# facebookresearch/metamorph

Hardware: AMD Instinct MI355X
Metric: train tokens/sec (LLaMA-3-8B + SigLIP-SO400M, seq2048, 256 img toks), whole job (higher is better)
Workload: dtype bf16

## Files before the change

metamorph_amd/csrc/attn.hip:

```cpp
#include "mm355_common.h"
#include "attn2.h"
#include <cstdlib>
#include <algorithm>

namespace {

constexpr int NT = 256;

__global__ __launch_bounds__(NT) void attn_delta_kernel(const uint16_t* __restrict__ o, const uint16_t* __restrict__ d_o, int64_t ld_o,
                                                        float* __restrict__ delta, int L, int Hq, int d) {
    const int l = blockIdx.x * 64 + (threadIdx.x >> 2), part = threadIdx.x & 3;
    const int h = blockIdx.y, b = blockIdx.z;
    const int dv = d >> 3;
    float s = 0.f;
    if (l < L) {
        for (int v = part; v < dv; v += 4) {
            float x[8], y[8];
            unpack8(*(const u32x4*)(o + ((int64_t)b * L + l) * ld_o + (int64_t)h * d + v * 8), x);
            unpack8(*(const u32x4*)(d_o + ((int64_t)b * L + l) * ld_o + (int64_t)h * d + v * 8), y);
#pragma unroll
            for (int e = 0; e < 8; ++e) s += x[e] * y[e];
        }
    }
    s += __shfl_xor(s, 1, 64);
// ... 72 lines not shown
    (void)hipGetLastError();
    if (!o || !d_o || !delta || B <= 0 || L <= 0 || Hq <= 0 || d <= 0 || d > 128 || (d & 7) || (ld_o & 7)) return MM355_EINVAL;
    dim3 grid((unsigned)((L + 63) / 64), (unsigned)Hq, (unsigned)B);
    hipLaunchKernelGGL(attn_delta_kernel, grid, dim3(NT), 0, (hipStream_t)stream, o, d_o, ld_o, delta, (int)L, (int)Hq, (int)d);
    return mm_launch_status();
}

extern "C" int64_t mm355_attn_bwd_ws_floats(int64_t B, int64_t L, int64_t Hq, int64_t Hkv, int64_t d, int64_t ld_max) {
    if (fast128(d, ld_max)) return 2 * B * Hq * L;
    if (Hq == Hkv) return 0;
    return 2 * B * L * Hq * d;
}

namespace {
int attn_bwd_impl(const mm355_bf16* q, const mm355_bf16* k, const mm355_bf16* v, int64_t ld_q, int64_t ld_k, const mm355_bf16* d_o,
                  int64_t ld_o, const float* lse, const float* delta, const int32_t* seqlens, mm355_bf16* dq, int64_t ld_dq,
                  mm355_bf16* dk, mm355_bf16* dv, int64_t ld_dkv, int64_t B, int64_t L, int64_t Hq, int64_t Hkv, int64_t d,
                  float scale, int causal, float* workspace, const uint16_t* rope_cos, const uint16_t* rope_sin, const int32_t* rope_pos,
                  int variant, void* stream) {
    (void)hipGetLastError();
    if (!q || !k || !v || !d_o || !lse || !delta || !dq || !dk || !dv || bad_geom(B, L, Hq, Hkv, d)) return MM355_EINVAL;
    if ((ld_q & 7) || (ld_k & 7) || (ld_o & 7) || (ld_dkv & 7) || (ld_dq & 7)) return MM355_EINVAL;
    const int64_t ld_max = std::max(std::max(ld_q, ld_k), ld_o);
    if (variant == 3) return MM355_EUNSUPPORTED;
    if (variant != 0 && variant != 2 && variant != 4 && variant != 41) return MM355_EINVAL;
    const bool is128 = fast128(d, ld_max) && variant != 2;
    const bool can4 = is128 && workspace && L * ld_max * 2 < 0x7fffffffll;
    if (is128 && !can4 && Hq != Hkv) return workspace ? MM355_EUNSUPPORTED : MM355_EINVAL;
    if (rope_cos && !can4) return MM355_EUNSUPPORTED;
    if ((variant == 4 || variant == 41) && !can4) return MM355_EUNSUPPORTED;
    if (variant == 4 || variant == 41 || (variant == 0 && can4)) {
        attn2::Args a4{q, k, v, d_o, ld_q, ld_k, ld_o, nullptr, nullptr, lse, delta, dq, ld_dq, seqlens,
                       dk, dv, nullptr, nullptr, ld_dkv, (int)B, (int)L, (int)Hq, (int)Hkv, (int)d, scale, causal, rope_cos, rope_sin, rope_pos};
        return mm355_attn4_bwd_launch(a4, workspace, variant == 41, (hipStream_t)stream);
    }
    if (Hq != Hkv && !workspace) return MM355_EINVAL;
    hipStream_t s = (hipStream_t)stream;
    float* dkp = nullptr;
    float* dvp = nullptr;
    if (Hq != Hkv) {
        dkp = workspace;
        dvp = workspace + (int64_t)B * L * Hq * d;
    }
    attn2::Args a{q, k, v, d_o, ld_q, ld_k, ld_o, nullptr, nullptr, lse, delta, dq, ld_dq, seqlens,
                  dk, dv, dkp, dvp, ld_dkv, (int)B, (int)L, (int)Hq, (int)Hkv, (int)d, scale, causal, rope_cos, rope_sin, rope_pos};
    int rc = mm355_attn2_dkdv_launch(a, pick_dp(d), s);
    if (rc != MM355_OK) return rc;
    if (dkp) {
        const int64_t rows = B * L;
        const unsigned rg = (unsigned)std::min<int64_t>((rows * (Hkv * d / 8) + NT - 1) / NT, 4096);
        hipLaunchKernelGGL(group_reduce_kernel, dim3(rg), dim3(NT), 0, s, dkp, dk, ld_dkv, rows, (int)Hq, (int)Hkv, (int)d);
        hipLaunchKernelGGL(group_reduce_kernel, dim3(rg), dim3(NT), 0, s, dvp, dv, ld_dkv, rows, (int)Hq, (int)Hkv, (int)d);
        rc = mm_launch_status();
        if (rc != MM355_OK) return rc;
    }
    return mm355_attn2_dq_launch(a, pick_dp(d), s);
}
}

extern "C" int mm355_attn_bwd(const mm355_bf16* q, const mm355_bf16* k, const mm355_bf16* v, int64_t ld_q, int64_t ld_k, const mm355_bf16* d_o,
                              int64_t ld_o, const float* lse, const float* delta, const int32_t* seqlens, mm355_bf16* dq, int64_t ld_dq,
                              mm355_bf16* dk, mm355_bf16* dv, int64_t ld_dkv, int64_t B, int64_t L, int64_t Hq, int64_t Hkv, int64_t d,
                              float scale, int causal, float* workspace, void* stream) {
    return attn_bwd_impl(q, k, v, ld_q, ld_k, d_o, ld_o, lse, delta, seqlens, dq, ld_dq, dk, dv, ld_dkv, B, L, Hq, Hkv, d, scale, causal, workspace,
                         nullptr, nullptr, nullptr, 0, stream);
}

// ... 20 lines not shown
```

metamorph_amd/csrc/attn4_bwd.hip:

```cpp
#include "attn2.h"

#ifndef ATTN4B_GEN_DIR
#define ATTN4B_GEN_DIR attn4_bwd_gen
#endif
#define ATTN4B_STR2(x) #x
#define ATTN4B_STR(x) ATTN4B_STR2(x)
#define ATTN4B_INC(f) ATTN4B_STR(ATTN4B_GEN_DIR/f)

namespace attn4b {
using namespace attn2;

constexpr float LOG2E = 1.4426950408889634f;
constexpr int SLOT = 32768;
constexpr int KV_BASE = 2048;
constexpr int KV_LDS = KV_BASE + 4 * SLOT, Q_LDS = 4 * SLOT;

MM_DEV int rot4(int row) { return ((row & 3) << 2) | ((row >> 2) & 3); }

struct LaneAddr {
    int RA[8], TA[4], TB[4], SA;
    MM_DEV void init(int lane) {
        const int c = lane & 31, hi = lane >> 5, g = lane >> 4, i = lane & 15;
#pragma unroll
        for (int ks = 0; ks < 8; ++ks) RA[ks] = c * 256 + (((ks * 2 + hi) ^ rot4(c)) << 4);
        const int row0 = 4 * hi + (i >> 2), row1 = row0 + 8;
#pragma unroll
        for (int db = 0; db < 4; ++db) {
            const int chunk = db * 4 + (g & 1) * 2 + ((i & 3) >> 1);
            TA[db] = row0 * 256 + ((chunk ^ rot4(row0)) << 4) + (i & 1) * 8;
            TB[db] = row1 * 256 + ((chunk ^ rot4(row1)) << 4) + (i & 1) * 8;
        }
        SA = hi * 16;
    }
};
MM_DEV void piece_offsets(int wave, int lane, uint32_t ldb, uint32_t (&vo)[4]) {
    const int r4 = lane >> 4, pc = lane & 15;
#pragma unroll
    for (int i = 0; i < 4; ++i) vo[i] = (uint32_t)(16 * wave + 4 * i + r4) * ldb + (uint32_t)((pc ^ ((r4 << 2) | i)) << 4);
}
MM_DEV uint32_t scale_pair(uint32_t w, float s) { return pack2bf(bflo(w) * s, bfhi(w) * s); }

#define BWD_BARRIER() asm volatile("s_waitcnt vmcnt(%0)\n\ts_barrier" :: "n"(NDMA) : "memory")

template <bool SAFE>
__global__ __launch_bounds__(256, 1) __attribute__((amdgpu_num_vgpr(96))) void dkdv_kernel(Args a, const float* __restrict__ nstat) {
    extern __shared__ __attribute__((aligned(16))) unsigned char smem[];
    asm volatile("" ::: "v255", "a255");
#ifdef MM355_ATTN4_TIMING
// ... 441 lines not shown
                for (int r = 0; r < 4; ++r) hi_[r] = x_[r] * keep;
            }
            if (a.rope_cos) {
                const int col = dbp * 32 + 8 * i4_ + 4 * hi;
                const u32x2 cw = *(const u32x2*)(a.rope_cos + (int64_t)pos * 128 + col);
                const u32x2 sw = *(const u32x2*)(a.rope_sin + (int64_t)pos * 128 + col);
                const float cs[4] = {bflo(cw.x), bfhi(cw.x), bflo(cw.y), bfhi(cw.y)};
                const float sn[4] = {bflo(sw.x), bfhi(sw.x), bflo(sw.y), bfhi(sw.y)};
#pragma unroll
                for (int r = 0; r < 4; ++r) {
                    const float x1 = round_bf(lo_[r]), x2 = round_bf(hi_[r]);
                    lo_[r] = x1 * cs[r] + x2 * sn[r];
                    hi_[r] = x2 * cs[r] - x1 * sn[r];
                }
            }
#pragma unroll
            for (int half = 0; half < 2; ++half) {
                const int db = dbp + 2 * half;
                const float* s4 = half ? hi_ : lo_;
                u32x2 w;
                w.x = pack2bf(s4[0], s4[1]);
                w.y = pack2bf(s4[2], s4[3]);
                *(u32x2*)(so + c * 256 + (((db * 4 + i4_) ^ (c & 15)) << 4) + hi * 8) = w;
            }
        }
    __syncthreads();
#pragma unroll
    for (int k = 0; k < 8; ++k) {
        const int r = 4 * k + (lane >> 4), j = lane & 15;
        if (qw0 + r < L) *(u32x4*)(dq_base + (int64_t)(qw0 + r) * a.ld_dq + j * 8) = *(const u32x4*)(so + r * 256 + ((j ^ (r & 15)) << 4));
    }
}

__global__ __launch_bounds__(256) void nstat_kernel(const float* __restrict__ lse, const float* __restrict__ delta, float* __restrict__ nstat, int64_t n,
                                                    float inv_scale) {
    for (int64_t i = blockIdx.x * 256ll + threadIdx.x; i < n; i += (int64_t)gridDim.x * 256) {
        nstat[i] = -lse[i] * inv_scale;
        nstat[n + i] = -delta[i];
    }
}

}

int mm355_attn4_bwd_launch(const attn2::Args& a, float* workspace, int variant, hipStream_t s) {
    static std::atomic<uint64_t> ok_kv{0}, ok_kvs{0}, ok_q{0}, ok_qs{0};
    const int64_t n = (int64_t)a.B * a.Hq * a.L;
    hipLaunchKernelGGL(attn4b::nstat_kernel, dim3((unsigned)std::min<int64_t>((n + 255) / 256, 2048)), dim3(256), 0, s, a.lse_in, a.delta, workspace, n, 1.0f / a.scale);
    const int64_t nkv = (int64_t)((a.L + 127) / 128) * a.Hkv * a.B, nq = (int64_t)((a.L + 127) / 128) * a.Hq * a.B;
    if (nkv > 0x7fffffff || nq > 0x7fffffff) return MM355_EINVAL;
    if (variant == 1) {
        if (mm_ensure_dynamic_lds((const void*)attn4b::dkdv_kernel<true>, attn4b::KV_LDS, ok_kvs) != MM355_OK) return MM355_ELAUNCH;
        if (mm_ensure_dynamic_lds((const void*)attn4b::dq_kernel<true>, attn4b::Q_LDS, ok_qs) != MM355_OK) return MM355_ELAUNCH;
        hipLaunchKernelGGL(attn4b::dkdv_kernel<true>, dim3((unsigned)nkv), dim3(256), attn4b::KV_LDS, s, a, (const float*)workspace);
        hipLaunchKernelGGL(attn4b::dq_kernel<true>, dim3((unsigned)nq), dim3(256), attn4b::Q_LDS, s, a);
    } else {
        if (mm_ensure_dynamic_lds((const void*)attn4b::dkdv_kernel<false>, attn4b::KV_LDS, ok_kv) != MM355_OK) return MM355_ELAUNCH;
        if (mm_ensure_dynamic_lds((const void*)attn4b::dq_kernel<false>, attn4b::Q_LDS, ok_q) != MM355_OK) return MM355_ELAUNCH;
        hipLaunchKernelGGL(attn4b::dkdv_kernel<false>, dim3((unsigned)nkv), dim3(256), attn4b::KV_LDS, s, a, (const float*)workspace);
        hipLaunchKernelGGL(attn4b::dq_kernel<false>, dim3((unsigned)nq), dim3(256), attn4b::Q_LDS, s, a);
    }
    return mm_launch_status();
}
```

Measured before the change: 26680.

## Pair causal dQ query blocks into one persistent workgroup for load balance

Adds a pair_dq_kernel in which each workgroup handles two query blocks: one near the end and one near the start of the causal sequence. This balances the triangular work per block and halves the grid, and the second block's Q/dO is prefetched into spare accumulator registers while the first is still running. The KV tile DMA pipeline runs across both blocks without restarting. The default variant 0 path now uses this kernel, while variant 4 keeps the old dq_kernel. The kernel depends on hand-written asm with fixed register assignments and occupancy 1, so it carries a correctness risk.

```diff
diff --git a/metamorph_amd/csrc/attn.hip b/metamorph_amd/csrc/attn.hip
--- a/metamorph_amd/csrc/attn.hip
+++ b/metamorph_amd/csrc/attn.hip
@@ -128,7 +128,7 @@
     if (variant == 4 || variant == 41 || (variant == 0 && can4)) {
         attn2::Args a4{q, k, v, d_o, ld_q, ld_k, ld_o, nullptr, nullptr, lse, delta, dq, ld_dq, seqlens,
                        dk, dv, nullptr, nullptr, ld_dkv, (int)B, (int)L, (int)Hq, (int)Hkv, (int)d, scale, causal, rope_cos, rope_sin, rope_pos};
-        return mm355_attn4_bwd_launch(a4, workspace, variant == 41, (hipStream_t)stream);
+        return mm355_attn4_bwd_launch(a4, workspace, variant, (hipStream_t)stream);
     }
     if (Hq != Hkv && !workspace) return MM355_EINVAL;
     hipStream_t s = (hipStream_t)stream;
diff --git a/metamorph_amd/csrc/attn4_bwd.hip b/metamorph_amd/csrc/attn4_bwd.hip
--- a/metamorph_amd/csrc/attn4_bwd.hip
+++ b/metamorph_amd/csrc/attn4_bwd.hip
@@ -13,7 +13,7 @@
 constexpr float LOG2E = 1.4426950408889634f;
 constexpr int SLOT = 32768;
 constexpr int KV_BASE = 2048;
-constexpr int KV_LDS = KV_BASE + 4 * SLOT, Q_LDS = 4 * SLOT;
+constexpr int KV_LDS = KV_BASE + 4 * SLOT, Q_LDS = 4 * SLOT, QP_LDS = Q_LDS + SLOT;
 
 MM_DEV int rot4(int row) { return ((row & 3) << 2) | ((row >> 2) & 3); }
 
@@ -521,6 +521,242 @@
     }
 }
 
+__global__ __launch_bounds__(256, 1) __attribute__((amdgpu_num_vgpr(80))) void pair_dq_kernel(Args a) {
+    extern __shared__ __attribute__((aligned(16))) unsigned char smem[];
+    asm volatile("" ::: "v255", "a255");
+    constexpr int NDMA = 8;
+    const int tid = threadIdx.x, lane = tid & 63;
+    const int wave = __builtin_amdgcn_readfirstlane(tid >> 6);
+    const int nblk = (a.L + 127) / 128;
+    int xp, hq, b;
+    block_coords((nblk + 1) / 2, a.Hq, inner_heads(a.Hq, a.Hq / a.Hkv), false, xp, hq, b);
+    const int hk = hq / (a.Hq / a.Hkv);
+    const int L = a.L;
+    const int seqlen = a.seqlens ? min(a.seqlens[b], L) : L;
+    const int64_t row_base = (int64_t)b * L;
+    uint16_t* dq_base = a.dqb + row_base * a.ld_dq + (int64_t)hq * 128;
+    int q0 = (nblk - 1 - xp) * 128;
+    const int q0n = xp * 128;
+    bool pair = q0n < q0;
+#define QP_ZERO_BLOCK(q_) do { \
+        for (int v = tid; v < 128 * 16; v += 256) { \
+            const int r = v >> 4, cc = (v & 15) * 8; \
+            if ((q_) + r < L) *(u32x4*)(dq_base + (int64_t)((q_) + r) * a.ld_dq + cc) = u32x4{0u, 0u, 0u, 0u}; \
+        } } while (0)
+    if (pair && q0n >= seqlen) { QP_ZERO_BLOCK(q0n); pair = false; }
+    if (q0 >= seqlen) {
+        QP_ZERO_BLOCK(q0);
+        if (!pair) return;
+        q0 = q0n; pair = false;
+    }
+#undef QP_ZERO_BLOCK
+    const int n1 = ((a.causal ? min(seqlen, q0 + 128) : seqlen) + 63) >> 6;
+    const int n2 = pair ? ((a.causal ? min(seqlen, q0n + 128) : seqlen) + 63) >> 6 : 0;
+    const uint32_t ldb = (uint32_t)a.ld_k * 2u;
+    const uint16_t* kbase = a.k + row_base * a.ld_k + (int64_t)hk * 128;
+    const uint16_t* vbase = a.v + row_base * a.ld_k + (int64_t)hk * 128;
+    const uint32_t nrec = (uint32_t)(seqlen - 1) * ldb + 256u;
+    const int64_t stat_row = ((int64_t)b * a.Hq + hq) * L;
+
+    const uint32_t sl2b_ = __builtin_amdgcn_readfirstlane(__float_as_uint(a.scale * LOG2E));
+    LaneAddr la;
+    la.init(lane);
+    int RA[8], TA[4], TB[4], RAH[8], TAH[4], TBH[4];
+#pragma unroll
+    for (int i = 0; i < 8; ++i) { RA[i] = la.RA[i]; RAH[i] = RA[i] + 65536; asm volatile("" : "+v"(RA[i])); asm volatile("" : "+v"(RAH[i])); }
+#pragma unroll
+    for (int i = 0; i < 4; ++i) {
+        TA[i] = la.TA[i]; TB[i] = la.TB[i]; TAH[i] = TA[i] + 65536; TBH[i] = TB[i] + 65536;
+        asm volatile("" : "+v"(TA[i])); asm volatile("" : "+v"(TB[i])); asm volatile("" : "+v"(TAH[i])); asm volatile("" : "+v"(TBH[i]));
+    }
+    uint32_t kvo[4];
+    piece_offsets(wave, lane, ldb, kvo);
+#pragma unroll
+    for (int i = 0; i < 4; ++i) asm volatile("" : "+v"(kvo[i]));
+    const float ninf = -INFINITY;
+#define QP_LANE(c_, hi_) int l_ = lane; asm volatile("" : "+v"(l_)); const int c_ = l_ & 31, hi_ = l_ >> 5
+    int qw0, qg, mlim_base, mlim_ = 0;
+    bool mask_cur = false;
+#define QP_BLOCK_VARS() do { \
+        QP_LANE(c_, hi_); \
+        qw0 = q0 + 32 * wave; qg = qw0 + c_; \
+        const int kmax_ = qg >= seqlen ? -1 : (a.causal ? min(qg, seqlen - 1) : seqlen - 1); \
+        mlim_base = kmax_ - 4 * hi_; } while (0)
+    QP_BLOCK_VARS();
+
+    __amdgpu_buffer_rsrc_t rsK, rsV;
+    int dst0 = 0, dt = 0, ct = 0;
+#define QP_TILE_VARS() do { \
+        const int t_ = dt < n1 ? dt : dt - n1; \
+        const uint32_t rec_ = dt < n1 + n2 ? nrec - (uint32_t)t_ * 64u * ldb : 0u; \
+        rsK = __builtin_amdgcn_make_buffer_rsrc((void*)(kbase + (int64_t)t_ * 64 * a.ld_k), 0, rec_, 0x00020000); \
+        rsV = __builtin_amdgcn_make_buffer_rsrc((void*)(vbase + (int64_t)t_ * 64 * a.ld_k), 0, rec_, 0x00020000); \
+        dst0 = (dt & 3) * SLOT; ++dt; } while (0)
+#define BWD_DMA(i) do { __builtin_amdgcn_sched_barrier(0); \
+        if ((i) < 4) __builtin_amdgcn_raw_ptr_buffer_load_lds(rsK, (lptr_t)(smem + dst0 + (wave * 4 + (i)) * 1024), 16, kvo[(i) & 3], 0, 0, 0); \
+        else __builtin_amdgcn_raw_ptr_buffer_load_lds(rsV, (lptr_t)(smem + dst0 + 16384 + (wave * 4 + (i) - 4) * 1024), 16, kvo[(i) & 3], 0, 0, 0); \
+        __builtin_amdgcn_sched_barrier(0); } while (0)
+
+    QP_TILE_VARS();
+#pragma unroll
+    for (int i = 0; i < 8; ++i) { BWD_DMA(i); }
+    QP_TILE_VARS();
+#pragma unroll
+    for (int i = 0; i < 8; ++i) { BWD_DMA(i); }
+    {
+        const int hi_ = lane >> 5;
+        const int qc = min(qg, L - 1);
+        const uint16_t* p0_ = a.q + (row_base + qc) * a.ld_q + (int64_t)hq * 128 + hi_ * 8;
+        const uint16_t* p1_ = a.d_o + (row_base + qc) * a.ld_o + (int64_t)hq * 128 + hi_ * 8;
+#include ATTN4B_INC(q_pers_load.inc)
+        const float nl_ = -a.lse_in[stat_row + qc] * (1.0f / a.scale);
+        const float nd_ = -a.delta[stat_row + qc];
+#include ATTN4B_INC(q_tuple_write.inc)
+    }
+#include ATTN4B_INC(q_zero.inc)
+    asm volatile("s_waitcnt vmcnt(0)" ::: "memory");
+    {
+        float t0_, t1_;
+#include ATTN4B_INC(q_pers_place.inc)
+    }
+    __builtin_amdgcn_s_barrier();
+
+    int gb = 0, n_tot = n1;
+    for (;;) {
+        QP_TILE_VARS();
+        switch ((gb + 3) & 3) {
+        case 0:
+#include ATTN4B_INC(q_head0.inc)
+            break;
+        case 1:
+#include ATTN4B_INC(q_head1.inc)
+            break;
+        case 2:
+#include ATTN4B_INC(q_head2.inc)
+            break;
+        default:
+#include ATTN4B_INC(q_head.inc)
+            break;
+        }
+        for (int u = 0; u < n_tot - 1; ++u) {
+            if (pair && u == n_tot - 2) {
+                QP_LANE(c_, hi_);
+                const int qc = min(q0n + 32 * wave + c_, L - 1);
+                const uint16_t* p0_ = a.q + (row_base + qc) * a.ld_q + (int64_t)hq * 128 + hi_ * 8;
+                const uint16_t* p1_ = a.d_o + (row_base + qc) * a.ld_o + (int64_t)hq * 128 + hi_ * 8;
+#include ATTN4B_INC(q_pair_load.inc)
+            }
+            QP_TILE_VARS(); Q_MASK_VARS();
+            switch ((gb + u) & 3) {
+            case 0:
+#include ATTN4B_INC(q_loop0.inc)
+                break;
+            case 1:
+#include ATTN4B_INC(q_loop1.inc)
+                break;
+            case 2:
+#include ATTN4B_INC(q_loop2.inc)
+                break;
+            default:
+#include ATTN4B_INC(q_loop3.inc)
+                break;
+            }
+        }
+        float lse2 = 0.0f, del2 = 0.0f;
+        if (pair) {
+            QP_LANE(c_, hi_);
+            (void)hi_;
+            const int qc = min(q0n + 32 * wave + c_, L - 1);
+            lse2 = a.lse_in[stat_row + qc];
+            del2 = a.delta[stat_row + qc];
+        }
+        Q_MASK_VARS();
+        switch ((gb + n_tot - 1) & 3) {
+        case 0:
+#include ATTN4B_INC(q_tail0.inc)
+            break;
+        case 1:
+#include ATTN4B_INC(q_tail1.inc)
+            break;
+        case 2:
+#include ATTN4B_INC(q_tail2.inc)
+            break;
+        default:
+#include ATTN4B_INC(q_tail3.inc)
+            break;
+        }
+        asm volatile("s_nop 15\n\ts_nop 15\n\ts_nop 15\n\ts_nop 15\n\ts_waitcnt vmcnt(0) lgkmcnt(0)" : "+v"(lse2), "+v"(del2) :: "memory");
+
+        QP_LANE(ce_, he_);
+        unsigned char* so = smem + Q_LDS + wave * 8192;
+        const float keep = qg < seqlen ? a.scale : 0.0f;
+        const int pos = min(qg, L - 1) + (a.rope_pos ? a.rope_pos[b] : 0);
+#pragma unroll
+        for (int dbp = 0; dbp < 2; ++dbp)
+#pragma unroll
+            for (int i4_ = 0; i4_ < 4; ++i4_) {
+                constexpr int which_ = 0;
+                float x_[4], lo_[4], hi_[4];
+                {
+                    const int db_ = dbp;
+#include ATTN4B_INC(q_acc_read.inc)
+#pragma unroll
+                    for (int r = 0; r < 4; ++r) lo_[r] = x_[r] * keep;
+                }
+                {
+                    const int db_ = dbp + 2;
+#include ATTN4B_INC(q_acc_read.inc)
+#pragma unroll
+                    for (int r = 0; r < 4; ++r) hi_[r] = x_[r] * keep;
+                }
+                if (a.rope_cos) {
+                    const int col = dbp * 32 + 8 * i4_ + 4 * he_;
+                    const u32x2 cw = *(const u32x2*)(a.rope_cos + (int64_t)pos * 128 + col);
+                    const u32x2 sw = *(const u32x2*)(a.rope_sin + (int64_t)pos * 128 + col);
+                    const float cs[4] = {bflo(cw.x), bfhi(cw.x), bflo(cw.y), bfhi(cw.y)};
+                    const float sn[4] = {bflo(sw.x), bfhi(sw.x), bflo(sw.y), bfhi(sw.y)};
+#pragma unroll
+                    for (int r = 0; r < 4; ++r) {
+                        const float x1 = round_bf(lo_[r]), x2 = round_bf(hi_[r]);
+                        lo_[r] = x1 * cs[r] + x2 * sn[r];
+                        hi_[r] = x2 * cs[r] - x1 * sn[r];
+                    }
+                }
+#pragma unroll
+                for (int half = 0; half < 2; ++half) {
+                    const int db = dbp + 2 * half;
+                    const float* s4 = half ? hi_ : lo_;
+                    u32x2 w;
+                    w.x = pack2bf(s4[0], s4[1]);
+                    w.y = pack2bf(s4[2], s4[3]);
+                    *(u32x2*)(so + ce_ * 256 + (((db * 4 + i4_) ^ (ce_ & 15)) << 4) + he_ * 8) = w;
+                }
+            }
+#pragma unroll
+        for (int k = 0; k < 8; ++k) {
+            const int r = 4 * k + (l_ >> 4), j = l_ & 15;
+            if (qw0 + r < L) *(u32x4*)(dq_base + (int64_t)(qw0 + r) * a.ld_dq + j * 8) = *(const u32x4*)(so + r * 256 + ((j ^ (r & 15)) << 4));
+        }
+        if (!pair) break;
+
+        {
+            const float nl_ = -lse2 * (1.0f / a.scale);
+            const float nd_ = -del2;
+#include ATTN4B_INC(q_zero.inc)
+#include ATTN4B_INC(q_pair_place.inc)
+#include ATTN4B_INC(q_tuple_write.inc)
+        }
+        asm volatile("s_nop 7" ::: "memory");
+        q0 = q0n; pair = false;
+        QP_BLOCK_VARS();
+        gb = n1; n_tot = n2; ct = 0;
+    }
+#undef BWD_DMA
+#undef QP_TILE_VARS
+#undef QP_BLOCK_VARS
+#undef QP_LANE
+}
+
 __global__ __launch_bounds__(256) void nstat_kernel(const float* __restrict__ lse, const float* __restrict__ delta, float* __restrict__ nstat, int64_t n,
                                                     float inv_scale) {
     for (int64_t i = blockIdx.x * 256ll + threadIdx.x; i < n; i += (int64_t)gridDim.x * 256) {
@@ -532,21 +768,27 @@
 }
 
 int mm355_attn4_bwd_launch(const attn2::Args& a, float* workspace, int variant, hipStream_t s) {
-    static std::atomic<uint64_t> ok_kv{0}, ok_kvs{0}, ok_q{0}, ok_qs{0};
+    static std::atomic<uint64_t> ok_kv{0}, ok_kvs{0}, ok_q{0}, ok_qs{0}, ok_qp{0};
     const int64_t n = (int64_t)a.B * a.Hq * a.L;
     hipLaunchKernelGGL(attn4b::nstat_kernel, dim3((unsigned)std::min<int64_t>((n + 255) / 256, 2048)), dim3(256), 0, s, a.lse_in, a.delta, workspace, n, 1.0f / a.scale);
-    const int64_t nkv = (int64_t)((a.L + 127) / 128) * a.Hkv * a.B, nq = (int64_t)((a.L + 127) / 128) * a.Hq * a.B;
+    const int64_t nblk = (a.L + 127) / 128;
+    const int64_t nkv = nblk * a.Hkv * a.B, nq = nblk * a.Hq * a.B, nqp = ((nblk + 1) / 2) * a.Hq * a.B;
     if (nkv > 0x7fffffff || nq > 0x7fffffff) return MM355_EINVAL;
-    if (variant == 1) {
+    if (variant == 41) {
         if (mm_ensure_dynamic_lds((const void*)attn4b::dkdv_kernel<true>, attn4b::KV_LDS, ok_kvs) != MM355_OK) return MM355_ELAUNCH;
         if (mm_ensure_dynamic_lds((const void*)attn4b::dq_kernel<true>, attn4b::Q_LDS, ok_qs) != MM355_OK) return MM355_ELAUNCH;
         hipLaunchKernelGGL(attn4b::dkdv_kernel<true>, dim3((unsigned)nkv), dim3(256), attn4b::KV_LDS, s, a, (const float*)workspace);
         hipLaunchKernelGGL(attn4b::dq_kernel<true>, dim3((unsigned)nq), dim3(256), attn4b::Q_LDS, s, a);
     } else {
         if (mm_ensure_dynamic_lds((const void*)attn4b::dkdv_kernel<false>, attn4b::KV_LDS, ok_kv) != MM355_OK) return MM355_ELAUNCH;
-        if (mm_ensure_dynamic_lds((const void*)attn4b::dq_kernel<false>, attn4b::Q_LDS, ok_q) != MM355_OK) return MM355_ELAUNCH;
         hipLaunchKernelGGL(attn4b::dkdv_kernel<false>, dim3((unsigned)nkv), dim3(256), attn4b::KV_LDS, s, a, (const float*)workspace);
-        hipLaunchKernelGGL(attn4b::dq_kernel<false>, dim3((unsigned)nq), dim3(256), attn4b::Q_LDS, s, a);
+        if (variant == 4) {
+            if (mm_ensure_dynamic_lds((const void*)attn4b::dq_kernel<false>, attn4b::Q_LDS, ok_q) != MM355_OK) return MM355_ELAUNCH;
+            hipLaunchKernelGGL(attn4b::dq_kernel<false>, dim3((unsigned)nq), dim3(256), attn4b::Q_LDS, s, a);
+        } else {
+            if (mm_ensure_dynamic_lds((const void*)attn4b::pair_dq_kernel, attn4b::QP_LDS, ok_qp) != MM355_OK) return MM355_ELAUNCH;
+            hipLaunchKernelGGL(attn4b::pair_dq_kernel, dim3((unsigned)nqp), dim3(256), attn4b::QP_LDS, s, a);
+        }
     }
     return mm_launch_status();
 }
diff --git a/metamorph_amd/csrc/attn4_bwd_gen/q_head0.inc b/metamorph_amd/csrc/attn4_bwd_gen/q_head0.inc
--- /dev/null
+++ b/metamorph_amd/csrc/attn4_bwd_gen/q_head0.inc
@@ -0,0 +1,114 @@
+asm volatile("ds_read_b128 a[128:131], %0 offset:32768" :  : "v"(RA[0]));
+asm volatile("ds_read_b128 a[132:135], %0 offset:40960" :  : "v"(RA[0]));
+asm volatile("ds_read_b128 a[136:139], %0 offset:49152" :  : "v"(RA[0]));
+asm volatile("ds_read_b128 a[140:143], %0 offset:57344" :  : "v"(RA[0]));
+asm volatile("ds_read_b128 a[144:147], %0 offset:32768" :  : "v"(RA[1]));
+asm volatile("ds_read_b128 a[148:151], %0 offset:40960" :  : "v"(RA[1]));
+asm volatile("ds_read_b128 a[152:155], %0 offset:49152" :  : "v"(RA[1]));
+asm volatile("ds_read_b128 a[156:159], %0 offset:57344" :  : "v"(RA[1]));
+asm volatile("s_waitcnt lgkmcnt(7)");
+asm volatile("v_mfma_f32_32x32x16_bf16 v[144:159], a[128:131], a[64:67], v[224:239]");
+asm volatile("ds_read_b128 a[128:131], %0 offset:32768" :  : "v"(RA[2]));
+asm volatile("s_waitcnt lgkmcnt(7)");
+asm volatile("v_mfma_f32_32x32x16_bf16 v[160:175], a[132:135], a[64:67], v[224:239]");
+asm volatile("ds_read_b128 a[132:135], %0 offset:40960" :  : "v"(RA[2]));
+BWD_DMA(0);
+asm volatile("s_waitcnt lgkmcnt(7)");
+asm volatile("v_mfma_f32_32x32x16_bf16 v[176:191], a[136:139], a[96:99], v[240:255]");
+asm volatile("ds_read_b128 a[136:139], %0 offset:49152" :  : "v"(RA[2]));
+BWD_DMA(1);
+asm volatile("s_waitcnt lgkmcnt(7)");
+asm volatile("v_mfma_f32_32x32x16_bf16 v[192:207], a[140:143], a[96:99], v[240:255]");
+asm volatile("ds_read_b128 a[140:143], %0 offset:57344" :  : "v"(RA[2]));
+BWD_DMA(2);
+asm volatile("s_waitcnt lgkmcnt(7)");
+asm volatile("v_mfma_f32_32x32x16_bf16 v[144:159], a[144:147], a[68:71], v[144:159]");
+asm volatile("ds_read_b128 a[144:147], %0 offset:32768" :  : "v"(RA[3]));
+BWD_DMA(3);
+asm volatile("s_waitcnt lgkmcnt(7)");
+asm volatile("v_mfma_f32_32x32x16_bf16 v[160:175], a[148:151], a[68:71], v[160:175]");
+asm volatile("ds_read_b128 a[148:151], %0 offset:40960" :  : "v"(RA[3]));
+BWD_DMA(4);
+asm volatile("s_waitcnt lgkmcnt(7)");
+asm volatile("v_mfma_f32_32x32x16_bf16 v[176:191], a[152:155], a[100:103], v[176:191]");
+asm volatile("ds_read_b128 a[152:155], %0 offset:49152" :  : "v"(RA[3]));
+BWD_DMA(5);
+asm volatile("s_waitcnt lgkmcnt(7)");
+asm volatile("v_mfma_f32_32x32x16_bf16 v[192:207], a[156:159], a[100:103], v[192:207]");
+asm volatile("ds_read_b128 a[156:159], %0 offset:57344" :  : "v"(RA[3]));
+BWD_DMA(6);
+asm volatile("s_waitcnt lgkmcnt(7)");
+asm volatile("v_mfma_f32_32x32x16_bf16 v[144:159], a[128:131], a[72:75], v[144:159]");
+asm volatile("ds_read_b128 a[128:131], %0 offset:32768" :  : "v"(RA[4]));
+BWD_DMA(7);
+asm volatile("s_waitcnt lgkmcnt(7)");
+asm volatile("v_mfma_f32_32x32x16_bf16 v[160:175], a[132:135], a[72:75], v[160:175]");
+asm volatile("ds_read_b128 a[132:135], %0 offset:40960" :  : "v"(RA[4]));
+asm volatile("s_waitcnt lgkmcnt(7)");
+asm volatile("v_mfma_f32_32x32x16_bf16 v[176:191], a[136:139], a[104:107], v[176:191]");
+asm volatile("ds_read_b128 a[136:139], %0 offset:49152" :  : "v"(RA[4]));
+asm volatile("s_waitcnt lgkmcnt(7)");
+asm volatile("v_mfma_f32_32x32x16_bf16 v[192:207], a[140:143], a[104:107], v[192:207]");
+asm volatile("ds_read_b128 a[140:143], %0 offset:57344" :  : "v"(RA[4]));
+asm volatile("s_waitcnt lgkmcnt(7)");
+asm volatile("v_mfma_f32_32x32x16_bf16 v[144:159], a[144:147], a[76:79], v[144:159]");
+asm volatile("ds_read_b128 a[144:147], %0 offset:32768" :  : "v"(RA[5]));
+asm volatile("s_waitcnt lgkmcnt(7)");
+asm volatile("v_mfma_f32_32x32x16_bf16 v[160:175], a[148:151], a[76:79], v[160:175]");
+asm volatile("ds_read_b128 a[148:151], %0 offset:40960" :  : "v"(RA[5]));
+asm volatile("s_waitcnt lgkmcnt(7)");
+asm volatile("v_mfma_f32_32x32x16_bf16 v[176:191], a[152:155], a[108:111], v[176:191]");
+asm volatile("ds_read_b128 a[152:155], %0 offset:49152" :  : "v"(RA[5]));
+asm volatile("s_waitcnt lgkmcnt(7)");
+asm volatile("v_mfma_f32_32x32x16_bf16 v[192:207], a[156:159], a[108:111], v[192:207]");
+asm volatile("ds_read_b128 a[156:159], %0 offset:57344" :  : "v"(RA[5]));
+asm volatile("s_waitcnt lgkmcnt(7)");
+asm volatile("v_mfma_f32_32x32x16_bf16 v[144:159], a[128:131], a[80:83], v[144:159]");
+asm volatile("ds_read_b128 a[128:131], %0 offset:32768" :  : "v"(RA[6]));
+asm volatile("s_waitcnt lgkmcnt(7)");
+asm volatile("v_mfma_f32_32x32x16_bf16 v[160:175], a[132:135], a[80:83], v[160:175]");
+asm volatile("ds_read_b128 a[132:135], %0 offset:40960" :  : "v"(RA[6]));
+asm volatile("s_waitcnt lgkmcnt(7)");
+asm volatile("v_mfma_f32_32x32x16_bf16 v[176:191], a[136:139], a[112:115], v[176:191]");
+asm volatile("ds_read_b128 a[136:139], %0 offset:49152" :  : "v"(RA[6]));
+asm volatile("s_waitcnt lgkmcnt(7)");
+asm volatile("v_mfma_f32_32x32x16_bf16 v[192:207], a[140:143], a[112:115], v[192:207]");
+asm volatile("ds_read_b128 a[140:143], %0 offset:57344" :  : "v"(RA[6]));
+asm volatile("s_waitcnt lgkmcnt(7)");
+asm volatile("v_mfma_f32_32x32x16_bf16 v[144:159], a[144:147], a[84:87], v[144:159]");
+asm volatile("ds_read_b128 a[144:147], %0 offset:32768" :  : "v"(RA[7]));
+asm volatile("s_waitcnt lgkmcnt(7)");
+asm volatile("v_mfma_f32_32x32x16_bf16 v[160:175], a[148:151], a[84:87], v[160:175]");
+asm volatile("ds_read_b128 a[148:151], %0 offset:40960" :  : "v"(RA[7]));
+asm volatile("s_waitcnt lgkmcnt(7)");
+asm volatile("v_mfma_f32_32x32x16_bf16 v[176:191], a[152:155], a[116:119], v[176:191]");
+asm volatile("ds_read_b128 a[152:155], %0 offset:49152" :  : "v"(RA[7]));
+asm volatile("s_waitcnt lgkmcnt(7)");
+asm volatile("v_mfma_f32_32x32x16_bf16 v[192:207], a[156:159], a[116:119], v[192:207]");
+asm volatile("ds_read_b128 a[156:159], %0 offset:57344" :  : "v"(RA[7]));
+asm volatile("s_waitcnt lgkmcnt(7)");
+asm volatile("v_mfma_f32_32x32x16_bf16 v[144:159], a[128:131], a[88:91], v[144:159]");
+asm volatile("s_waitcnt lgkmcnt(6)");
+asm volatile("v_mfma_f32_32x32x16_bf16 v[160:175], a[132:135], a[88:91], v[160:175]");
+asm volatile("s_waitcnt lgkmcnt(5)");
+asm volatile("v_mfma_f32_32x32x16_bf16 v[176:191], a[136:139], a[120:123], v[176:191]");
+asm volatile("s_waitcnt lgkmcnt(4)");
+asm volatile("v_mfma_f32_32x32x16_bf16 v[192:207], a[140:143], a[120:123], v[192:207]");
+asm volatile("s_waitcnt lgkmcnt(3)");
+asm volatile("v_mfma_f32_32x32x16_bf16 v[144:159], a[144:147], a[92:95], v[144:159]");
+asm volatile("s_waitcnt lgkmcnt(2)");
+asm volatile("v_mfma_f32_32x32x16_bf16 v[160:175], a[148:151], a[92:95], v[160:175]");
+asm volatile("s_waitcnt lgkmcnt(1)");
+asm volatile("v_mfma_f32_32x32x16_bf16 v[176:191], a[152:155], a[124:127], v[176:191]");
+asm volatile("s_waitcnt lgkmcnt(0)");
+asm volatile("v_mfma_f32_32x32x16_bf16 v[192:207], a[156:159], a[124:127], v[192:207]");
+asm volatile("s_nop 15\n\ts_nop 15");
+BWD_BARRIER();
+asm volatile("ds_read_b128 a[128:131], %0 offset:0" :  : "v"(RAH[0]));
+asm volatile("ds_read_b128 a[132:135], %0 offset:8192" :  : "v"(RAH[0]));
+asm volatile("ds_read_b128 a[136:139], %0 offset:16384" :  : "v"(RAH[0]));
+asm volatile("ds_read_b128 a[140:143], %0 offset:24576" :  : "v"(RAH[0]));
+asm volatile("ds_read_b128 a[144:147], %0 offset:0" :  : "v"(RAH[1]));
+asm volatile("ds_read_b128 a[148:151], %0 offset:8192" :  : "v"(RAH[1]));
+asm volatile("ds_read_b128 a[152:155], %0 offset:16384" :  : "v"(RAH[1]));
+asm volatile("ds_read_b128 a[156:159], %0 offset:24576" :  : "v"(RAH[1]));
diff --git a/metamorph_amd/csrc/attn4_bwd_gen/q_head1.inc b/metamorph_amd/csrc/attn4_bwd_gen/q_head1.inc
--- /dev/null
+++ b/metamorph_amd/csrc/attn4_bwd_gen/q_head1.inc
@@ -0,0 +1,114 @@
+asm volatile("ds_read_b128 a[128:131], %0 offset:0" :  : "v"(RAH[0]));
+asm volatile("ds_read_b128 a[132:135], %0 offset:8192" :  : "v"(RAH[0]));
+asm volatile("ds_read_b128 a[136:139], %0 offset:16384" :  : "v"(RAH[0]));
+asm volatile("ds_read_b128 a[140:143], %0 offset:24576" :  : "v"(RAH[0]));
+asm volatile("ds_read_b128 a[144:147], %0 offset:0" :  : "v"(RAH[1]));
+asm volatile("ds_read_b128 a[148:151], %0 offset:8192" :  : "v"(RAH[1]));
+asm volatile("ds_read_b128 a[152:155], %0 offset:16384" :  : "v"(RAH[1]));
+asm volatile("ds_read_b128 a[156:159], %0 offset:24576" :  : "v"(RAH[1]));
+asm volatile("s_waitcnt lgkmcnt(7)");
+asm volatile("v_mfma_f32_32x32x16_bf16 v[80:95], a[128:131], a[64:67], v[224:239]");
+asm volatile("ds_read_b128 a[128:131], %0 offset:0" :  : "v"(RAH[2]));
+asm volatile("s_waitcnt lgkmcnt(7)");
+asm volatile("v_mfma_f32_32x32x16_bf16 v[96:111], a[132:135], a[64:67], v[224:239]");
+asm volatile("ds_read_b128 a[132:135], %0 offset:8192" :  : "v"(RAH[2]));
+BWD_DMA(0);
+asm volatile("s_waitcnt lgkmcnt(7)");
+asm volatile("v_mfma_f32_32x32x16_bf16 v[112:127], a[136:139], a[96:99], v[240:255]");
+asm volatile("ds_read_b128 a[136:139], %0 offset:16384" :  : "v"(RAH[2]));
+BWD_DMA(1);
+asm volatile("s_waitcnt lgkmcnt(7)");
+asm volatile("v_mfma_f32_32x32x16_bf16 v[128:143], a[140:143], a[96:99], v[240:255]");
+asm volatile("ds_read_b128 a[140:143], %0 offset:24576" :  : "v"(RAH[2]));
+BWD_DMA(2);
+asm volatile("s_waitcnt lgkmcnt(7)");
+asm volatile("v_mfma_f32_32x32x16_bf16 v[80:95], a[144:147], a[68:71], v[80:95]");
+asm volatile("ds_read_b128 a[144:147], %0 offset:0" :  : "v"(RAH[3]));
+BWD_DMA(3);
+asm volatile("s_waitcnt lgkmcnt(7)");
+asm volatile("v_mfma_f32_32x32x16_bf16 v[96:111], a[148:151], a[68:71], v[96:111]");
+asm volatile("ds_read_b128 a[148:151], %0 offset:8192" :  : "v"(RAH[3]));
+BWD_DMA(4);
+asm volatile("s_waitcnt lgkmcnt(7)");
+asm volatile("v_mfma_f32_32x32x16_bf16 v[112:127], a[152:155], a[100:103], v[112:127]");
+asm volatile("ds_read_b128 a[152:155], %0 offset:16384" :  : "v"(RAH[3]));
+BWD_DMA(5);
+asm volatile("s_waitcnt lgkmcnt(7)");
+asm volatile("v_mfma_f32_32x32x16_bf16 v[128:143], a[156:159], a[100:103], v[128:143]");
+asm volatile("ds_read_b128 a[156:159], %0 offset:24576" :  : "v"(RAH[3]));
+BWD_DMA(6);
+asm volatile("s_waitcnt lgkmcnt(7)");
+asm volatile("v_mfma_f32_32x32x16_bf16 v[80:95], a[128:131], a[72:75], v[80:95]");
+asm volatile("ds_read_b128 a[128:131], %0 offset:0" :  : "v"(RAH[4]));
+BWD_DMA(7);
+asm volatile("s_waitcnt lgkmcnt(7)");
+asm volatile("v_mfma_f32_32x32x16_bf16 v[96:111], a[132:135], a[72:75], v[96:111]");
+asm volatile("ds_read_b128 a[132:135], %0 offset:8192" :  : "v"(RAH[4]));
+asm volatile("s_waitcnt lgkmcnt(7)");
+asm volatile("v_mfma_f32_32x32x16_bf16 v[112:127], a[136:139], a[104:107], v[112:127]");
+asm volatile("ds_read_b128 a[136:139], %0 offset:16384" :  : "v"(RAH[4]));
+asm volatile("s_waitcnt lgkmcnt(7)");
+asm volatile("v_mfma_f32_32x32x16_bf16 v[128:143], a[140:143], a[104:107], v[128:143]");
+asm volatile("ds_read_b128 a[140:143], %0 offset:24576" :  : "v"(RAH[4]));
+asm volatile("s_waitcnt lgkmcnt(7)");
+asm volatile("v_mfma_f32_32x32x16_bf16 v[80:95], a[144:147], a[76:79], v[80:95]");
+asm volatile("ds_read_b128 a[144:147], %0 offset:0" :  : "v"(RAH[5]));
+asm volatile("s_waitcnt lgkmcnt(7)");
+asm volatile("v_mfma_f32_32x32x16_bf16 v[96:111], a[148:151], a[76:79], v[96:111]");
+asm volatile("ds_read_b128 a[148:151], %0 offset:8192" :  : "v"(RAH[5]));
+asm volatile("s_waitcnt lgkmcnt(7)");
+asm volatile("v_mfma_f32_32x32x16_bf16 v[112:127], a[152:155], a[108:111], v[112:127]");
+asm volatile("ds_read_b128 a[152:155], %0 offset:16384" :  : "v"(RAH[5]));
+asm volatile("s_waitcnt lgkmcnt(7)");
+asm volatile("v_mfma_f32_32x32x16_bf16 v[128:143], a[156:159], a[108:111], v[128:143]");
+asm volatile("ds_read_b128 a[156:159], %0 offset:24576" :  : "v"(RAH[5]));
+asm volatile("s_waitcnt lgkmcnt(7)");
+asm volatile("v_mfma_f32_32x32x16_bf16 v[80:95], a[128:131], a[80:83], v[80:95]");
+asm volatile("ds_read_b128 a[128:131], %0 offset:0" :  : "v"(RAH[6]));
+asm volatile("s_waitcnt lgkmcnt(7)");
+asm volatile("v_mfma_f32_32x32x16_bf16 v[96:111], a[132:135], a[80:83], v[96:111]");
+asm volatile("ds_read_b128 a[132:135], %0 offset:8192" :  : "v"(RAH[6]));
+asm volatile("s_waitcnt lgkmcnt(7)");
+asm volatile("v_mfma_f32_32x32x16_bf16 v[112:127], a[136:139], a[112:115], v[112:127]");
+asm volatile("ds_read_b128 a[136:139], %0 offset:16384" :  : "v"(RAH[6]));
+asm volatile("s_waitcnt lgkmcnt(7)");
+asm volatile("v_mfma_f32_32x32x16_bf16 v[128:143], a[140:143], a[112:115], v[128:143]");
+asm volatile("ds_read_b128 a[140:143], %0 offset:24576" :  : "v"(RAH[6]));
+asm volatile("s_waitcnt lgkmcnt(7)");
+asm volatile("v_mfma_f32_32x32x16_bf16 v[80:95], a[144:147], a[84:87], v[80:95]");
+asm volatile("ds_read_b128 a[144:147], %0 offset:0" :  : "v"(RAH[7]));
+asm volatile("s_waitcnt lgkmcnt(7)");
+asm volatile("v_mfma_f32_32x32x16_bf16 v[96:111], a[148:151], a[84:87], v[96:111]");
+asm volatile("ds_read_b128 a[148:151], %0 offset:8192" :  : "v"(RAH[7]));
+asm volatile("s_waitcnt lgkmcnt(7)");
+asm volatile("v_mfma_f32_32x32x16_bf16 v[112:127], a[152:155], a[116:119], v[112:127]");
+asm volatile("ds_read_b128 a[152:155], %0 offset:16384" :  : "v"(RAH[7]));
+asm volatile("s_waitcnt lgkmcnt(7)");
+asm volatile("v_mfma_f32_32x32x16_bf16 v[128:143], a[156:159], a[116:119], v[128:143]");
+asm volatile("ds_read_b128 a[156:159], %0 offset:24576" :  : "v"(RAH[7]));
+asm volatile("s_waitcnt lgkmcnt(7)");
+asm volatile("v_mfma_f32_32x32x16_bf16 v[80:95], a[128:131], a[88:91], v[80:95]");
+asm volatile("s_waitcnt lgkmcnt(6)");
+asm volatile("v_mfma_f32_32x32x16_bf16 v[96:111], a[132:135], a[88:91], v[96:111]");
+asm volatile("s_waitcnt lgkmcnt(5)");
+asm volatile("v_mfma_f32_32x32x16_bf16 v[112:127], a[136:139], a[120:123], v[112:127]");
+asm volatile("s_waitcnt lgkmcnt(4)");
+asm volatile("v_mfma_f32_32x32x16_bf16 v[128:143], a[140:143], a[120:123], v[128:143]");
+asm volatile("s_waitcnt lgkmcnt(3)");
+asm volatile("v_mfma_f32_32x32x16_bf16 v[80:95], a[144:147], a[92:95], v[80:95]");
+asm volatile("s_waitcnt lgkmcnt(2)");
+asm volatile("v_mfma_f32_32x32x16_bf16 v[96:111], a[148:151], a[92:95], v[96:111]");
+asm volatile("s_waitcnt lgkmcnt(1)");
+asm volatile("v_mfma_f32_32x32x16_bf16 v[112:127], a[152:155], a[124:127], v[112:127]");
+asm volatile("s_waitcnt lgkmcnt(0)");
+asm volatile("v_mfma_f32_32x32x16_bf16 v[128:143], a[156:159], a[124:127], v[128:143]");
+asm volatile("s_nop 15\n\ts_nop 15");
+BWD_BARRIER();
+asm volatile("ds_read_b128 a[128:131], %0 offset:32768" :  : "v"(RAH[0]));
+asm volatile("ds_read_b128 a[132:135], %0 offset:40960" :  : "v"(RAH[0]));
+asm volatile("ds_read_b128 a[136:139], %0 offset:49152" :  : "v"(RAH[0]));
+asm volatile("ds_read_b128 a[140:143], %0 offset:57344" :  : "v"(RAH[0]));
+asm volatile("ds_read_b128 a[144:147], %0 offset:32768" :  : "v"(RAH[1]));
+asm volatile("ds_read_b128 a[148:151], %0 offset:40960" :  : "v"(RAH[1]));
+asm volatile("ds_read_b128 a[152:155], %0 offset:49152" :  : "v"(RAH[1]));
+asm volatile("ds_read_b128 a[156:159], %0 offset:57344" :  : "v"(RAH[1]));
diff --git a/metamorph_amd/csrc/attn4_bwd_gen/q_head2.inc b/metamorph_amd/csrc/attn4_bwd_gen/q_head2.inc
--- /dev/null
+++ b/metamorph_amd/csrc/attn4_bwd_gen/q_head2.inc
@@ -0,0 +1,114 @@
+asm volatile("ds_read_b128 a[128:131], %0 offset:32768" :  : "v"(RAH[0]));
+asm volatile("ds_read_b128 a[132:135], %0 offset:40960" :  : "v"(RAH[0]));
+asm volatile("ds_read_b128 a[136:139], %0 offset:49152" :  : "v"(RAH[0]));
+asm volatile("ds_read_b128 a[140:143], %0 offset:57344" :  : "v"(RAH[0]));
+asm volatile("ds_read_b128 a[144:147], %0 offset:32768" :  : "v"(RAH[1]));
+asm volatile("ds_read_b128 a[148:151], %0 offset:40960" :  : "v"(RAH[1]));
+asm volatile("ds_read_b128 a[152:155], %0 offset:49152" :  : "v"(RAH[1]));
+asm volatile("ds_read_b128 a[156:159], %0 offset:57344" :  : "v"(RAH[1]));
+asm volatile("s_waitcnt lgkmcnt(7)");
+asm volatile("v_mfma_f32_32x32x16_bf16 v[144:159], a[128:131], a[64:67], v[224:239]");
+asm volatile("ds_read_b128 a[128:131], %0 offset:32768" :  : "v"(RAH[2]));
+asm volatile("s_waitcnt lgkmcnt(7)");
+asm volatile("v_mfma_f32_32x32x16_bf16 v[160:175], a[132:135], a[64:67], v[224:239]");
+asm volatile("ds_read_b128 a[132:135], %0 offset:40960" :  : "v"(RAH[2]));
+BWD_DMA(0);
+asm volatile("s_waitcnt lgkmcnt(7)");
+asm volatile("v_mfma_f32_32x32x16_bf16 v[176:191], a[136:139], a[96:99], v[240:255]");
+asm volatile("ds_read_b128 a[136:139], %0 offset:49152" :  : "v"(RAH[2]));
+BWD_DMA(1);
+asm volatile("s_waitcnt lgkmcnt(7)");
+asm volatile("v_mfma_f32_32x32x16_bf16 v[192:207], a[140:143], a[96:99], v[240:255]");
+asm volatile("ds_read_b128 a[140:143], %0 offset:57344" :  : "v"(RAH[2]));
+BWD_DMA(2);
+asm volatile("s_waitcnt lgkmcnt(7)");
+asm volatile("v_mfma_f32_32x32x16_bf16 v[144:159], a[144:147], a[68:71], v[144:159]");
+asm volatile("ds_read_b128 a[144:147], %0 offset:32768" :  : "v"(RAH[3]));
+BWD_DMA(3);
+asm volatile("s_waitcnt lgkmcnt(7)");
+asm volatile("v_mfma_f32_32x32x16_bf16 v[160:175], a[148:151], a[68:71], v[160:175]");
+asm volatile("ds_read_b128 a[148:151], %0 offset:40960" :  : "v"(RAH[3]));
+BWD_DMA(4);
+asm volatile("s_waitcnt lgkmcnt(7)");
+asm volatile("v_mfma_f32_32x32x16_bf16 v[176:191], a[152:155], a[100:103], v[176:191]");
+asm volatile("ds_read_b128 a[152:155], %0 offset:49152" :  : "v"(RAH[3]));
+BWD_DMA(5);
+asm volatile("s_waitcnt lgkmcnt(7)");
+asm volatile("v_mfma_f32_32x32x16_bf16 v[192:207], a[156:159], a[100:103], v[192:207]");
+asm volatile("ds_read_b128 a[156:159], %0 offset:57344" :  : "v"(RAH[3]));
+BWD_DMA(6);
+asm volatile("s_waitcnt lgkmcnt(7)");
+asm volatile("v_mfma_f32_32x32x16_bf16 v[144:159], a[128:131], a[72:75], v[144:159]");
+asm volatile("ds_read_b128 a[128:131], %0 offset:32768" :  : "v"(RAH[4]));
+BWD_DMA(7);
+asm volatile("s_waitcnt lgkmcnt(7)");
+asm volatile("v_mfma_f32_32x32x16_bf16 v[160:175], a[132:135], a[72:75], v[160:175]");
+asm volatile("ds_read_b128 a[132:135], %0 offset:40960" :  : "v"(RAH[4]));
+asm volatile("s_waitcnt lgkmcnt(7)");
+asm volatile("v_mfma_f32_32x32x16_bf16 v[176:191], a[136:139], a[104:107], v[176:191]");
+asm volatile("ds_read_b128 a[136:139], %0 offset:49152" :  : "v"(RAH[4]));
+asm volatile("s_waitcnt lgkmcnt(7)");
+asm volatile("v_mfma_f32_32x32x16_bf16 v[192:207], a[140:143], a[104:107], v[192:207]");
+asm volatile("ds_read_b128 a[140:143], %0 offset:57344" :  : "v"(RAH[4]));
+asm volatile("s_waitcnt lgkmcnt(7)");
+asm volatile("v_mfma_f32_32x32x16_bf16 v[144:159], a[144:147], a[76:79], v[144:159]");
+asm volatile("ds_read_b128 a[144:147], %0 offset:32768" :  : "v"(RAH[5]));
+asm volatile("s_waitcnt lgkmcnt(7)");
+asm volatile("v_mfma_f32_32x32x16_bf16 v[160:175], a[148:151], a[76:79], v[160:175]");
+asm volatile("ds_read_b128 a[148:151], %0 offset:40960" :  : "v"(RAH[5]));
+asm volatile("s_waitcnt lgkmcnt(7)");
+asm volatile("v_mfma_f32_32x32x16_bf16 v[176:191], a[152:155], a[108:111], v[176:191]");
+asm volatile("ds_read_b128 a[152:155], %0 offset:49152" :  : "v"(RAH[5]));
+asm volatile("s_waitcnt lgkmcnt(7)");
+asm volatile("v_mfma_f32_32x32x16_bf16 v[192:207], a[156:159], a[108:111], v[192:207]");
+asm volatile("ds_read_b128 a[156:159], %0 offset:57344" :  : "v"(RAH[5]));
+asm volatile("s_waitcnt lgkmcnt(7)");
+asm volatile("v_mfma_f32_32x32x16_bf16 v[144:159], a[128:131], a[80:83], v[144:159]");
+asm volatile("ds_read_b128 a[128:131], %0 offset:32768" :  : "v"(RAH[6]));
+asm volatile("s_waitcnt lgkmcnt(7)");
+asm volatile("v_mfma_f32_32x32x16_bf16 v[160:175], a[132:135], a[80:83], v[160:175]");
+asm volatile("ds_read_b128 a[132:135], %0 offset:40960" :  : "v"(RAH[6]));
+asm volatile("s_waitcnt lgkmcnt(7)");
+asm volatile("v_mfma_f32_32x32x16_bf16 v[176:191], a[136:139], a[112:115], v[176:191]");
+asm volatile("ds_read_b128 a[136:139], %0 offset:49152" :  : "v"(RAH[6]));
+asm volatile("s_waitcnt lgkmcnt(7)");
+asm volatile("v_mfma_f32_32x32x16_bf16 v[192:207], a[140:143], a[112:115], v[192:207]");
+asm volatile("ds_read_b128 a[140:143], %0 offset:57344" :  : "v"(RAH[6]));
+asm volatile("s_waitcnt lgkmcnt(7)");
+asm volatile("v_mfma_f32_32x32x16_bf16 v[144:159], a[144:147], a[84:87], v[144:159]");
+asm volatile("ds_read_b128 a[144:147], %0 offset:32768" :  : "v"(RAH[7]));
+asm volatile("s_waitcnt lgkmcnt(7)");
+asm volatile("v_mfma_f32_32x32x16_bf16 v[160:175], a[148:151], a[84:87], v[160:175]");
+asm volatile("ds_read_b128 a[148:151], %0 offset:40960" :  : "v"(RAH[7]));
+asm volatile("s_waitcnt lgkmcnt(7)");
+asm volatile("v_mfma_f32_32x32x16_bf16 v[176:191], a[152:155], a[116:119], v[176:191]");
+asm volatile("ds_read_b128 a[152:155], %0 offset:49152" :  : "v"(RAH[7]));
+asm volatile("s_waitcnt lgkmcnt(7)");
+asm volatile("v_mfma_f32_32x32x16_bf16 v[192:207], a[156:159], a[116:119], v[192:207]");
+asm volatile("ds_read_b128 a[156:159], %0 offset:57344" :  : "v"(RAH[7]));
+asm volatile("s_waitcnt lgkmcnt(7)");
+asm volatile("v_mfma_f32_32x32x16_bf16 v[144:159], a[128:131], a[88:91], v[144:159]");
+asm volatile("s_waitcnt lgkmcnt(6)");
+asm volatile("v_mfma_f32_32x32x16_bf16 v[160:175], a[132:135], a[88:91], v[160:175]");
+asm volatile("s_waitcnt lgkmcnt(5)");
+asm volatile("v_mfma_f32_32x32x16_bf16 v[176:191], a[136:139], a[120:123], v[176:191]");
+asm volatile("s_waitcnt lgkmcnt(4)");
+asm volatile("v_mfma_f32_32x32x16_bf16 v[192:207], a[140:143], a[120:123], v[192:207]");
+asm volatile("s_waitcnt lgkmcnt(3)");
+asm volatile("v_mfma_f32_32x32x16_bf16 v[144:159], a[144:147], a[92:95], v[144:159]");
+asm volatile("s_waitcnt lgkmcnt(2)");
+asm volatile("v_mfma_f32_32x32x16_bf16 v[160:175], a[148:151], a[92:95], v[160:175]");
+asm volatile("s_waitcnt lgkmcnt(1)");
+asm volatile("v_mfma_f32_32x32x16_bf16 v[176:191], a[152:155], a[124:127], v[176:191]");
+asm volatile("s_waitcnt lgkmcnt(0)");
+asm volatile("v_mfma_f32_32x32x16_bf16 v[192:207], a[156:159], a[124:127], v[192:207]");
+asm volatile("s_nop 15\n\ts_nop 15");
+BWD_BARRIER();
+asm volatile("ds_read_b128 a[128:131], %0 offset:0" :  : "v"(RA[0]));
+asm volatile("ds_read_b128 a[132:135], %0 offset:8192" :  : "v"(RA[0]));
+asm volatile("ds_read_b128 a[136:139], %0 offset:16384" :  : "v"(RA[0]));
+asm volatile("ds_read_b128 a[140:143], %0 offset:24576" :  : "v"(RA[0]));
+asm volatile("ds_read_b128 a[144:147], %0 offset:0" :  : "v"(RA[1]));
+asm volatile("ds_read_b128 a[148:151], %0 offset:8192" :  : "v"(RA[1]));
+asm volatile("ds_read_b128 a[152:155], %0 offset:16384" :  : "v"(RA[1]));
+asm volatile("ds_read_b128 a[156:159], %0 offset:24576" :  : "v"(RA[1]));
diff --git a/metamorph_amd/csrc/attn4_bwd_gen/q_pair_load.inc b/metamorph_amd/csrc/attn4_bwd_gen/q_pair_load.inc
--- /dev/null
+++ b/metamorph_amd/csrc/attn4_bwd_gen/q_pair_load.inc
@@ -0,0 +1,2 @@
+asm volatile("global_load_dwordx4 a[192:195], %0, off offset:0\n\tglobal_load_dwordx4 a[196:199], %0, off offset:32\n\tglobal_load_dwordx4 a[200:203], %0, off offset:64\n\tglobal_load_dwordx4 a[204:207], %0, off offset:96\n\tglobal_load_dwordx4 a[208:211], %0, off offset:128\n\tglobal_load_dwordx4 a[212:215], %0, off offset:160\n\tglobal_load_dwordx4 a[216:219], %0, off offset:192\n\tglobal_load_dwordx4 a[220:223], %0, off offset:224" :  : "v"(p0_) : "memory");
+asm volatile("global_load_dwordx4 a[224:227], %0, off offset:0\n\tglobal_load_dwordx4 a[228:231], %0, off offset:32\n\tglobal_load_dwordx4 a[232:235], %0, off offset:64\n\tglobal_load_dwordx4 a[236:239], %0, off offset:96\n\tglobal_load_dwordx4 a[240:243], %0, off offset:128\n\tglobal_load_dwordx4 a[244:247], %0, off offset:160\n\tglobal_load_dwordx4 a[248:251], %0, off offset:192\n\tglobal_load_dwordx4 a[252:255], %0, off offset:224" :  : "v"(p1_) : "memory");
diff --git a/metamorph_amd/csrc/attn4_bwd_gen/q_pair_place.inc b/metamorph_amd/csrc/attn4_bwd_gen/q_pair_place.inc
--- /dev/null
+++ b/metamorph_amd/csrc/attn4_bwd_gen/q_pair_place.inc
@@ -0,0 +1,64 @@
+asm volatile("v_accvgpr_mov_b32 a64, a192");
+asm volatile("v_accvgpr_mov_b32 a65, a193");
+asm volatile("v_accvgpr_mov_b32 a66, a194");
+asm volatile("v_accvgpr_mov_b32 a67, a195");
+asm volatile("v_accvgpr_mov_b32 a68, a196");
+asm volatile("v_accvgpr_mov_b32 a69, a197");
+asm volatile("v_accvgpr_mov_b32 a70, a198");
+asm volatile("v_accvgpr_mov_b32 a71, a199");
+asm volatile("v_accvgpr_mov_b32 a72, a200");
+asm volatile("v_accvgpr_mov_b32 a73, a201");
+asm volatile("v_accvgpr_mov_b32 a74, a202");
+asm volatile("v_accvgpr_mov_b32 a75, a203");
+asm volatile("v_accvgpr_mov_b32 a76, a204");
+asm volatile("v_accvgpr_mov_b32 a77, a205");
+asm volatile("v_accvgpr_mov_b32 a78, a206");
+asm volatile("v_accvgpr_mov_b32 a79, a207");
+asm volatile("v_accvgpr_mov_b32 a80, a208");
+asm volatile("v_accvgpr_mov_b32 a81, a209");
+asm volatile("v_accvgpr_mov_b32 a82, a210");
+asm volatile("v_accvgpr_mov_b32 a83, a211");
+asm volatile("v_accvgpr_mov_b32 a84, a212");
+asm volatile("v_accvgpr_mov_b32 a85, a213");
+asm volatile("v_accvgpr_mov_b32 a86, a214");
+asm volatile("v_accvgpr_mov_b32 a87, a215");
+asm volatile("v_accvgpr_mov_b32 a88, a216");
+asm volatile("v_accvgpr_mov_b32 a89, a217");
+asm volatile("v_accvgpr_mov_b32 a90, a218");
+asm volatile("v_accvgpr_mov_b32 a91, a219");
+asm volatile("v_accvgpr_mov_b32 a92, a220");
+asm volatile("v_accvgpr_mov_b32 a93, a221");
+asm volatile("v_accvgpr_mov_b32 a94, a222");
+asm volatile("v_accvgpr_mov_b32 a95, a223");
+asm volatile("v_accvgpr_mov_b32 a96, a224");
+asm volatile("v_accvgpr_mov_b32 a97, a225");
+asm volatile("v_accvgpr_mov_b32 a98, a226");
+asm volatile("v_accvgpr_mov_b32 a99, a227");
+asm volatile("v_accvgpr_mov_b32 a100, a228");
+asm volatile("v_accvgpr_mov_b32 a101, a229");
+asm volatile("v_accvgpr_mov_b32 a102, a230");
+asm volatile("v_accvgpr_mov_b32 a103, a231");
+asm volatile("v_accvgpr_mov_b32 a104, a232");
+asm volatile("v_accvgpr_mov_b32 a105, a233");
+asm volatile("v_accvgpr_mov_b32 a106, a234");
+asm volatile("v_accvgpr_mov_b32 a107, a235");
+asm volatile("v_accvgpr_mov_b32 a108, a236");
+asm volatile("v_accvgpr_mov_b32 a109, a237");
+asm volatile("v_accvgpr_mov_b32 a110, a238");
+asm volatile("v_accvgpr_mov_b32 a111, a239");
+asm volatile("v_accvgpr_mov_b32 a112, a240");
+asm volatile("v_accvgpr_mov_b32 a113, a241");
+asm volatile("v_accvgpr_mov_b32 a114, a242");
+asm volatile("v_accvgpr_mov_b32 a115, a243");
+asm volatile("v_accvgpr_mov_b32 a116, a244");
+asm volatile("v_accvgpr_mov_b32 a117, a245");
+asm volatile("v_accvgpr_mov_b32 a118, a246");
+asm volatile("v_accvgpr_mov_b32 a119, a247");
+asm volatile("v_accvgpr_mov_b32 a120, a248");
+asm volatile("v_accvgpr_mov_b32 a121, a249");
+asm volatile("v_accvgpr_mov_b32 a122, a250");
+asm volatile("v_accvgpr_mov_b32 a123, a251");
+asm volatile("v_accvgpr_mov_b32 a124, a252");
+asm volatile("v_accvgpr_mov_b32 a125, a253");
+asm volatile("v_accvgpr_mov_b32 a126, a254");
+asm volatile("v_accvgpr_mov_b32 a127, a255");
```

Measured after the change: 26610. Within noise of the previous version (-0.2%).
